# lks1248/SPH-EXA

Measured on AMD Instinct MI355X. Metric: particle-updates/sec (whole node), Sedov -n 400, 1/2/4/8 MI355X + HBM roofline %, higher is better.
Workload: dtype f32 hydro / f64 coordinates (sph::SphTypes)

## Files before the change

### sph-exa_amd/csrc/sx_sim.hpp

```cpp
#pragma once

#include <hip/hip_runtime.h>

#include <cmath>
#include <initializer_list>
#include <string>
#include <utility>
#include <vector>

#include "../../include/sphexa_hip.h"
#include "sx_comm.hpp"
#include "sx_hydro.hpp"
#include "sx_map.hpp"
#include "sx_profile.hpp"
#include "sx_fof.hpp"
#include "sx_twopoint.hpp"
#include "sx_spectrum.hpp"
#include "sx_step_timer.hpp"
#include "sx_tree.hpp"

namespace sx::turb
{
struct SimTurb;
}

namespace sx::sim
{

struct Scalars
{
    double   minDt, minDt_m1, ttot, minDtCourant, minDtRho;
    double   dtCand;
    float    courant;
    unsigned maxDivvU;
    double   egrav;
    unsigned long long maxAccSqBits;
    unsigned gravErr;
};

inline Scalars freshScalars(double minDt = 1e-6, double minDt_m1 = 1e-6)
{
    return Scalars{.minDt = minDt, .minDt_m1 = minDt_m1, .ttot = 0.0, .minDtCourant = INFINITY, .minDtRho = INFINITY,
                   .dtCand = 0.0, .courant = 1e10f, .maxDivvU = 0u, .egrav = 0.0, .maxAccSqBits = 0ull, .gravErr = 0u};
}

struct Fields
{
    double *  x, *y, *z, *temp;
    float *   h, *m, *vx, *vy, *vz, *xm1, *ym1, *zm1, *dum1, *alpha;
    uint64_t* id;
    uint8_t*  rung;
};

struct BdtState
{
    sx_timestep ts{}, prev{};
    bool        started{false};
    double      minDt{0}, minDt_m1{0}, ttot{0};
    float       searchExt{1.f};
    double      margin{1.05};
    double      egrav{0};
    uint64_t    haloShort{0};
    uint64_t    hierarchies{0}, warnedAt{~0ull};
    uint32_t*   groupBuf{nullptr};
    sx_groups   groups{}, tsGroups{}, active{}, rungs[SX_MAX_RUNGS]{};
    float*      groupDt{nullptr};
    uint32_t*   groupIdx{nullptr};
    uint32_t *  tsStart[2]{}, *tsEnd[2]{};
    uint8_t*    activeMask{nullptr};
    uint32_t*   maskRange{nullptr};
    uint64_t    substeps{0};
};

struct SkinState
{
    float    factor{0.05f};
    float    cur{0.05f};
    float    built{0.05f};
    int      maxReuse{24};
    float    staleLimit{0.125f};
    bool     valid{false};
    bool     forceBuild{false};
    int      sinceBuild{0};
    uint32_t ngmaxS{0};
    int      backoff{0}, backoffLen{4};
    int      cleanSinceBuild{0};
    uint64_t plainSteps{0};
    uint64_t builds{0}, reuseSteps{0}, staleClusters{0}, exactClusters{0};
    uint64_t resyncs{0};
    uint32_t lastStale{0}, lastExact{0};
    uint64_t stepClusters{0}, stepS13{0};
    bool      xmFused{false};
    uint32_t* exactList{nullptr};
    bool      listsKept{false};
    const void *keptNloc{nullptr}, *keptUni{nullptr}, *keptMask{nullptr}, *keptSame{nullptr}, *keptFrz{nullptr},
        *keptNlocB{nullptr};
    uint64_t  keptClusters{0}, frozenClusters{0};
    uint64_t  earlyExact{0};
    sx::ListsB lb{};
};


struct SkinBuffers
{
    float *   dx{nullptr}, *dy{nullptr}, *dz{nullptr};
    uint32_t* cells{nullptr};
    float *   rel{nullptr}, *hb{nullptr}, *acc{nullptr};
    uint32_t *sloc{nullptr}, *scnt{nullptr}, *ucountS{nullptr}, *l1{nullptr}, *l2{nullptr}, *l3{nullptr};
    uint8_t*  dec{nullptr};
    uint32_t* host{nullptr};
    uint8_t * streak{nullptr}, *same{nullptr};
    uint32_t* hitmask{nullptr};
    float2*   frz{nullptr};
    uint32_t *nlocB{nullptr}, *ucountB{nullptr}, *hitmaskB{nullptr};
    double *drift{nullptr}, *relg{nullptr}, *x0{nullptr}, *y0{nullptr}, *z0{nullptr};
    float* h0{nullptr};
};

struct ReqBox;

struct DomBuffers
{
    uint32_t* bins{nullptr};
    uint64_t *split{nullptr}, *seg{nullptr}, *cnth{nullptr};
    uint32_t *agree{nullptr}, *agreeh{nullptr};
    unsigned *hflag{nullptr}, *hflagh{nullptr};
    uint32_t* errh{nullptr};
    ReqBox*   mybox{nullptr};
};

struct GravBuffers
{
    unsigned long long* inter{nullptr};
    int32_t*            farL2N{nullptr};
    uint32_t*           farLay{nullptr};
};

}

struct sx_sim
{
    using Scalars = sx::sim::Scalars;
    using Fields  = sx::sim::Fields;

    sx_ctx*        ctx;
    sx::NsPolicy   nsPolicy;
    sx::Transport* comm{nullptr};
    sx_comm*       commHandle{nullptr};
    sx_params      p;
    sx_box         box;
    sx::DevBox     dbox;
    uint32_t       bucket;
    size_t         cap{0}, n{0}, first{0}, last{0};
    sx::Arena      mem;
    sx::Arena      work;
    sx::DevTree    tree;
    sx::DevTree    localTree;
    sx::Arena      farMem;
    sx::Arena      gravWork;
    sx::DevTree    farTree;
    sx::DevTree    nearTree;

    double *  x, *y, *z, *temp;
    float *   h, *m, *vx, *vy, *vz, *xm1, *ym1, *zm1, *dum1, *alpha;
    uint64_t* id;
    uint8_t*  rung{nullptr};
    uint64_t* keys;
    uint32_t *order, *nc;
    float *   xm, *kx, *gradh, *prho, *c, *divv, *curlv, *c11, *c12, *c13, *c22, *c23, *c33, *ax, *ay, *az;
    double*   du;
    float*    dV[6]{};
    float *   rho{nullptr}, *pres{nullptr};
    sx::RecX* rx;
    sx::RecV* rv;
    sx::RecT* rt;
    sx::RecS* rs;
    sx::RecC* rc;
    sx::NbLists nb;
    uint32_t* stats;
    uint32_t* statsHost;
    int       sortBits{30};
    bool      gravCount = false;
    uint32_t  gravCheckTargets{0};
    bool      gravCheckValid{false};
    double    gravCheck[6]{};
    bool      keysFresh = false;
    uint64_t  sortStats[4]{0, 0, 0, 0};
    Scalars*  sc;
    Scalars*  scHost;

    struct Spare
    {
        void** field;
        void*  alt;
        int    elemBytes;
    };
// ... 71 lines not shown
```

### sph-exa_amd/csrc/sx_sim_skin.cpp

```cpp
#include "sx_sim_internal.hpp"

using namespace sx;
using namespace sx::sim;

namespace
{

__global__ void coverListKernel(const uint32_t* list, uint32_t maxList, uint32_t first, uint32_t last, const double* x,
                                const double* y, const double* z, const float* r, float scale, const ReqBox* boxes,
                                DevBox box, double qmargin, const double* drift, const double* x0, const double* y0,
                                const double* z0, const double* relg, unsigned* flag)
{
    const uint32_t k = blockIdx.x;
    if (k >= min(list[0], maxList)) return;
    const uint32_t i = first + list[1 + k] * kCluster + threadIdx.x;
    if (i >= last) return;
    const ReqBox& b  = boxes[(i - first) / kChunk];
    const double  R  = 2.0 * (double)r[i] * (double)scale * (1.0 + 1e-6) + qmargin;
    const double  Ra = R + drift[0], Rr = R + relg[i];
    const bool    outNow = fabs(foldPbc(x[i] - b.c[0], box, 0)) + Ra > b.s[0] ||
                        fabs(foldPbc(y[i] - b.c[1], box, 1)) + Ra > b.s[1] ||
                        fabs(foldPbc(z[i] - b.c[2], box, 2)) + Ra > b.s[2];
    const bool    outBuild = fabs(foldPbc(x0[i] - b.c[0], box, 0)) + Rr > b.s[0] ||
                          fabs(foldPbc(y0[i] - b.c[1], box, 1)) + Rr > b.s[1] ||
// ... 58 lines not shown
void skinTooThin(SkinState& K)
{
    K.forceBuild = true;
    if (K.cur < kMaxSkin) K.cur = std::min(2.0f * K.cur, kMaxSkin);
    else
    {
        K.backoff    = K.backoffLen;
        K.backoffLen = std::min(2 * K.backoffLen, 32);
    }
}

SkinGrid skinGrid(const DevBox& b)
{
    SkinGrid g{};
    g.n = kSkinGridN;
    for (int d = 0; d < 3; ++d)
    {
        g.lo[d]  = b.lim[2 * d];
        g.inv[d] = (double)kSkinGridN / b.l[d];
        g.pbc[d] = b.pbc[d];
    }
    return g;
}

uint32_t skinCapacity(uint32_t ngmax, float factor)
{
    const double f = std::pow(1.0 + factor, 3.0) * 1.15;
    const uint32_t c = (uint32_t)std::ceil(ngmax * f);
    return std::min<uint32_t>(256u, (c + 1u) & ~1u);
}

static bool skinReserveDisp(sx_sim* s)
{
    auto& B = s->skinBuf;
    B.dx    = s->mem.get<float>("skin.dx", s->cap);
    B.dy    = s->mem.get<float>("skin.dy", s->cap);
    B.dz    = s->mem.get<float>("skin.dz", s->cap);
    B.cells = s->mem.get<uint32_t>("skin.cells", kGridWords * (size_t)kSkinGridN * kSkinGridN * kSkinGridN);
    return B.dx && B.dy && B.dz && B.cells;
}

static bool skinReserveDrift(sx_sim* s)
{
    auto& B = s->skinBuf;
    B.drift = s->mem.get<double>("skin.drift", 8);
    B.relg  = s->mem.get<double>("skin.relg", s->cap);
    B.x0    = s->mem.get<double>("skin.x0", s->cap);
    B.y0    = s->mem.get<double>("skin.y0", s->cap);
    B.z0    = s->mem.get<double>("skin.z0", s->cap);
    return B.drift && B.relg && B.x0 && B.y0 && B.z0;
}

bool skinParticleBuffers(sx_sim* s, PosArgs& q, hipStream_t st)
{
    const size_t nc = (size_t)kSkinGridN * kSkinGridN * kSkinGridN;
    const bool   ok = skinReserveDisp(s);
    const auto&  B  = s->skinBuf;
    q.dispX = B.dx, q.dispY = B.dy, q.dispZ = B.dz, q.cells = B.cells;
    q.grid  = skinGrid(s->dbox);
    if (!ok) return false;
    return hipMemsetAsync(q.cells, 0xff, 3 * nc * sizeof(uint32_t), st) == hipSuccess &&
           hipMemsetAsync(q.cells + 3 * nc, 0, 3 * nc * sizeof(uint32_t), st) == hipSuccess;
}

static bool skinReserveSearch(sx_sim* s, const NsArgs& na, uint32_t ncl, bool twoSets)
{
    auto&      B    = s->skinBuf;
    auto&      M    = s->mem;
    const bool disp = skinReserveDisp(s);
    B.rel     = M.get<float>("skin.rel", s->cap);
    B.sloc    = M.get<uint32_t>("skin.sloc", na.numGroups * (size_t)nlocWords(s->skin.ngmaxS) * kWave);
    B.scnt    = M.get<uint32_t>("skin.scnt", s->cap);
    B.hb      = M.get<float>("skin.hb", s->cap);
    B.acc     = M.get<float>("skin.acc", ncl);
    B.ucountS = M.get<uint32_t>("skin.ucount", ncl);
    B.l1      = M.get<uint32_t>("skin.l1", ncl + 1);
    B.l2      = M.get<uint32_t>("skin.l2", ncl + 1);
    B.l3      = M.get<uint32_t>("skin.l3", ncl + 1);
    B.dec     = M.get<uint8_t>("skin.dec", ncl);
    B.host    = M.pinned<uint32_t>("skin.host", 4);
    B.streak  = M.get<uint8_t>("skin.streak", ncl);
    B.hitmask = M.get<uint32_t>("skin.hitmask", na.numGroups * (size_t)kSkinMaskWords * kWave);
    B.same    = M.get<uint8_t>("skin.same", ncl);
    B.frz     = M.get<float2>("skin.frz", ncl);
    B.nlocB    = twoSets ? M.get<uint32_t>("skin.nlocB", na.numGroups * (size_t)nlocWords(na.ngmax) * kWave) : nullptr;
    B.ucountB  = twoSets ? M.get<uint32_t>("skin.ucountB", ncl) : nullptr;
    B.hitmaskB = twoSets ? M.get<uint32_t>("skin.hitmaskB", na.numGroups * (size_t)kSkinMaskWords * kWave) : nullptr;
    return disp && B.rel && B.sloc && B.scnt && B.hb && B.acc && B.ucountS && B.l1 && B.l2 && B.l3 && B.dec && B.host &&
           B.streak && B.hitmask && B.same && B.frz && (!twoSets || (B.nlocB && B.ucountB && B.hitmaskB));
}

int skinSearch(sx_sim* s, const NsArgs& na, bool reuse, hipStream_t st, float* xmOut, RecT* rtXm, SkinCounts& out)
{
    auto&          K   = s->skin;
    const uint32_t ncl = (na.numGroups + kClusterWaves - 1) / kClusterWaves;
    out                = SkinCounts{};
    out.clusters       = ncl;
    if (!reuse) K.built = K.cur;
    if (!ncl) return SX_OK;
    if (!reuse) K.ngmaxS = skinCapacity(s->p.ngmax, K.built);
    const bool twoSets = na.ucap / 4 >= (uint32_t)kSkinCap && !getenv("SX_SKIN_ONESET");
    if (!skinReserveSearch(s, na, ncl, twoSets)) return SX_ERR_NOMEM;
    const SkinBuffers& B = s->skinBuf;
    uint32_t *const l1 = B.l1, *const l2 = B.l2, *const l3 = B.l3, *const hl = B.host;
    uint32_t* const hmask = B.hitmask, *const nlocB = B.nlocB;
    uint8_t* const  same  = B.same;
    float2* const   frz   = B.frz;

    const SkinGrid g = skinGrid(s->dbox);
    SkinArgs fa{};
    fa.first = na.first, fa.last = na.last, fa.numGroups = na.numGroups, fa.ngmax = na.ngmax, fa.ng0 = na.ng0;
    fa.ngmaxS = K.ngmaxS, fa.iterateH = na.iterateH, fa.skin1 = 1.0f + K.built;
    fa.x = na.x, fa.y = na.y, fa.z = na.z, fa.h = na.h, fa.m = na.m, fa.nc = na.nc, fa.rxOut = na.rxOut;
    const uint32_t uoff = na.ucap / 2;
    fa.nloc = na.nloc, fa.uni = na.uni, fa.ucount = na.ucount, fa.ucap = na.ucap, fa.uoff = uoff, fa.ucountS = B.ucountS;
    fa.packMax = na.packMax;
    fa.sloc = B.sloc, fa.scnt = B.scnt, fa.hb = B.hb, fa.rel = B.rel, fa.acc = B.acc, fa.cells = B.cells, fa.grid = g;
    fa.dispX = B.dx, fa.dispY = B.dy, fa.dispZ = B.dz;
    fa.xmOut = xmOut, fa.rtXm = rtXm, fa.K = s->p.K;
    K.xmFused   = xmOut != nullptr;
    K.exactList = l2;
    fa.box = na.box, fa.powTab = na.powTab, fa.stats = na.stats, fa.clStats = na.clStats;
    fa.hitMask   = hmask;
    fa.same      = same;
    fa.nlocB = nlocB, fa.ucountB = B.ucountB, fa.hitMaskB = B.hitmaskB, fa.uoffB = na.ucap / 4;
    fa.frz       = getenv("SX_SKIN_NOFREEZE") ? nullptr : frz;
    fa.keepLists = reuse && K.listsKept && K.keptNloc == na.nloc && K.keptUni == na.uni && K.keptMask == hmask &&
                   K.keptSame == same && K.keptFrz == frz && K.keptNlocB == nlocB;
    K.listsKept  = false;

    NsArgs b   = na;
    b.skin1    = 1.0f + K.built;
    b.iterateH = 0;
    b.nloc     = B.sloc;
    b.packMax  = 0;
    b.ngmax    = K.ngmaxS;
    b.nc       = B.scnt;
    b.rxOut    = nullptr;
    b.uoff     = uoff;
    b.ucount   = B.ucountS;

    SIM_HIP(hipMemsetAsync(l1, 0, 4, st));
    SIM_HIP(hipMemsetAsync(l2, 0, 4, st));
    if (!reuse)
    {
        SIM_HIP(hipMemsetAsync(B.streak, 0, ncl, st));
        SIM_HIP(findNeighbors(b, st));
        fa.fresh = 1;
    }
    else fa.fresh = 0;
    fa.list  = nullptr;
    fa.stale = l1;
    fa.streak = reuse ? B.streak : nullptr;
    fa.direct = reuse ? l2 : nullptr;
    if (reuse)
    {
        fa.dec = B.dec;
        const char* fs = getenv("SX_SKIN_FROZEN_STAGE");
        fa.frozenStage = fs ? (uint32_t)std::max(0, atoi(fs)) : (uint32_t)kSkinFrozenCap;
        SIM_HIP(skinDecide(fa, ncl, st));
        SIM_HIP(skinFrozen(fa, ncl, st));
    }
    SIM_HIP(skinFilter(fa, ncl, st));
    SIM_HIP(hipMemcpyAsync(hl, l1, 4, hipMemcpyDeviceToHost, st));
    SIM_HIP(hipMemcpyAsync(hl + 1, l2, 4, hipMemcpyDeviceToHost, st));
    SIM_HIP(hipStreamSynchronize(st));
    const uint32_t n1 = hl[0], nd = hl[1];
    uint32_t       n2 = nd;
    out.rebuilt = n1, out.stale = n1 + nd, out.exact = nd;
    NsArgs         x  = na;
    NsPolicy large;
    large.mode = 1;
    if (reuse) b.policy = x.policy = &large;
    if ((n1 || nd) && reuse)
    {
        double* c3 = s->mem.get<double>("skin.centers", 3 * (size_t)s->tree.numNodes);
        double* s3 = s->mem.get<double>("skin.sizes", 3 * (size_t)s->tree.numNodes);
        if (!c3 || !s3) return SX_ERR_NOMEM;
        SIM_HIP(skinRefreshBoxes(s->tree, na.x, na.y, na.z, na.box, c3, s3, st));
        b.centers = x.centers = c3;
        b.sizes = x.sizes = s3;
    }
    const bool early = n1 && nd && reuse && s->auxStream && s->evAuxIn && s->evAuxOut && !getenv("SX_SKIN_SERIAL_EXACT");
    if (early)
    {
        NsArgs xd   = x;
        xd.subset   = l2;
        xd.work     = s->mem.get<uint32_t>("skin.aux.work", 16);
        xd.hSave    = s->mem.get<float>("skin.aux.over", ncl + 1);
        xd.hitMasks = s->mem.get<uint64_t>("skin.aux.masks", searchScratchBytes() / sizeof(uint64_t));
        const char* sh = getenv("SX_SKIN_AUX_SHARE");
        if (!sh || atoi(sh) != 0)
        {
            const unsigned G = searchGrid();
            xd.maxGrid       = std::min(nd, G / 2);
            b.maxGrid        = G - xd.maxGrid;
        }
        if (!xd.work || !xd.hSave || !xd.hitMasks) return SX_ERR_NOMEM;
        SIM_HIP(hipEventRecord(s->evAuxIn, st));
        SIM_HIP(hipStreamWaitEvent(s->auxStream, s->evAuxIn, 0));
        SIM_HIP(findNeighbors(xd, s->auxStream));
        SIM_HIP(hipEventRecord(s->evAuxOut, s->auxStream));
    }
    uint32_t* lx = l2;
    if (n1)
    {
        b.subset  = l1;
        SIM_HIP(findNeighbors(b, st));
        fa.fresh  = 1;
        fa.list   = l1;
        if (early) SIM_HIP(hipMemsetAsync(l3, 0, 4, st));
        fa.stale  = early ? l3 : l2;
        fa.streak = nullptr;
        fa.direct = nullptr;
        fa.dec    = nullptr;
        SIM_HIP(skinFilter(fa, ncl, st));
        SIM_HIP(hipMemcpyAsync(hl + 2, fa.stale, 4, hipMemcpyDeviceToHost, st));
        SIM_HIP(hipStreamSynchronize(st));
        n2 = hl[2];
    }
    uint32_t n3 = 0;
    if (early)
    {
        n3 = n2, n2 = nd + n3, lx = l3;
        K.earlyExact += nd;
        SIM_HIP(hipStreamWaitEvent(st, s->evAuxOut, 0));
    }
    out.exact = n2;
    {
        if (early ? n3 : n2)
        {
            x.subset = lx;
            SIM_HIP(findNeighbors(x, st));
        }
        if (early)
        {
            if (n3) SIM_HIP(hipMemcpyAsync(l2 + 1 + nd, l3 + 1, 4 * (size_t)n3, hipMemcpyDeviceToDevice, st));
            hl[3] = n2;
            SIM_HIP(hipMemcpyAsync(l2, hl + 3, 4, hipMemcpyHostToDevice, st));
        }
        if (n2)
        {
            if (reuse)
            {
                SIM_HIP(hipMemcpyAsync(hl, na.stats, 4, hipMemcpyDeviceToHost, st));
                SIM_HIP(hipStreamSynchronize(st));
                if (hl[0] & 1u)
                {
                    SIM_HIP(hipMemsetAsync(na.stats, 0, 4, st));
                    return kSkinResync;
                }
            }
            SIM_HIP(skinMarkStale(l2, ncl, B.acc, st));
        }
    }
    SIM_HIP(reduceClusterStats(na.clStats, ncl, na.stats, st));
    K.listsKept = true, K.keptNloc = na.nloc, K.keptUni = na.uni, K.keptMask = hmask, K.keptSame = same, K.keptFrz = frz;
    K.keptNlocB = nlocB;
    K.lb = twoSets ? ListsB{same, nlocB, B.ucountB, na.ucap / 4} : ListsB{};
    if (getenv("SX_SKIN_DEBUG"))
    {
        uint32_t f = 0;
        SIM_HIP(hipMemcpyAsync(&f, na.stats, 4, hipMemcpyDeviceToHost, st));
        SIM_HIP(hipStreamSynchronize(st));
        fprintf(stderr, "skin: reuse %d s %.3f clusters %u stale %u exact %u (direct %u) flags 0x%x mode %d\n",
                (int)reuse, K.built, ncl, n1 + nd, n2, nd, f, s->nsPolicy.mode);
    }
    return SX_OK;
}

void skinDecide(SkinState& K, bool reuse, const SkinCounts& c, uint64_t staleAll, uint64_t clustersAll)
{
    K.lastStale = c.stale, K.lastExact = c.exact;
    K.staleClusters += c.stale, K.exactClusters += c.exact;
    if (reuse)
    {
        K.reuseSteps++;
        K.sinceBuild++;
    }
    else
    {
        K.builds++;
        K.valid      = true;
        K.forceBuild = false;
        K.sinceBuild = 0;
    }
    const bool clean = (double)staleAll <= K.staleLimit * (double)clustersAll;
    if (!reuse) K.cleanSinceBuild = 0;
    else if (clean) K.cleanSinceBuild++;
    if (!clean)
    {
        K.forceBuild = true;
        if (!reuse || K.cleanSinceBuild < 2) skinTooThin(K);
        else if (K.sinceBuild < kShortSkin) K.cur = std::min(1.25f * K.cur, kMaxSkin);
    }
    if (clean && K.cleanSinceBuild >= 2) K.backoffLen = 4;
}

int skinHaloRefresh(sx_sim* s, hipStream_t st)
{
    if (int e = haloExchange(s, {{s->x, 8}, {s->y, 8}, {s->z, 8}, {s->h, 4}, {s->m, 4}}, st)) return e;
    const size_t nc = (size_t)kSkinGridN * kSkinGridN * kSkinGridN;
    const auto&  B  = s->skinBuf;
    if (!skinReserveDisp(s)) return SX_ERR_NOMEM;
    SIM_COMM(s->comm->allreduceMinU32(B.cells, 3 * nc, st));
    SIM_COMM(s->comm->allreduceMaxU32(B.cells + 3 * nc, 3 * nc, st));
    if (!skinReserveDrift(s)) return SX_ERR_NOMEM;
    uint32_t* red = reinterpret_cast<uint32_t*>(B.drift + 2);
    SIM_HIP(hipMemsetAsync(red, 0, 7 * 4, st));
    SIM_HIP(hipMemsetAsync(red + 1, 0xff, 3 * 4, st));
    skinGridMaxKernel<<<grid(nc), 256, 0, st>>>(B.cells, (uint32_t)nc, red);
    const size_t nl = s->last - s->first;
    skinDriftKernel<<<std::max(1u, grid(nl)), 256, 0, st>>>(red, (uint32_t)s->first, (uint32_t)s->last, B.dx, B.dy, B.dz,
                                                           B.drift, B.relg);
    SIM_HIP(hipGetLastError());
    return SX_OK;
}

int skinBuildSnapshot(sx_sim* s, hipStream_t st)
{
    if (!skinReserveDrift(s)) return SX_ERR_NOMEM;
    const auto&  B  = s->skinBuf;
    const size_t f0 = s->first, nl0 = s->last - s->first;
    SIM_HIP(hipMemsetAsync(B.drift, 0, 8 * sizeof(double), st));
    SIM_HIP(hipMemsetAsync(B.relg + f0, 0, nl0 * sizeof(double), st));
    double*       p0[3] = {B.x0, B.y0, B.z0};
    const double* pc[3] = {s->x, s->y, s->z};
    for (int d = 0; d < 3; ++d)
        SIM_HIP(hipMemcpyAsync(p0[d] + f0, pc[d] + f0, nl0 * sizeof(double), hipMemcpyDeviceToDevice, st));
    return SX_OK;
}

int skinCoverCheck(sx_sim* s, const SkinCounts& c, unsigned* flag, hipStream_t st)
{
    const auto& B = s->skinBuf;
    if (!B.drift || !B.relg || !B.x0 || !B.y0 || !B.z0) return SX_ERR_NOMEM;
    const double   qm    = quantMargin(s->dbox);
    const uint32_t first = (uint32_t)s->first, last = (uint32_t)s->last;
    if (c.rebuilt)
        coverListKernel<<<c.rebuilt, kCluster, 0, st>>>(B.l1, c.rebuilt, first, last, s->x, s->y, s->z, B.hb,
                                                        1.0f + s->skin.built, s->dom.mybox, s->dbox, qm, B.drift, B.x0,
// ... 18 lines not shown
```

### sph-exa_amd/csrc/sx_skin.hip

```cpp
#include "sx_kernel_poly.hpp"
#include "sx_skin.hpp"
#include "sx_traverse.hpp"

namespace sx
{

namespace
{

constexpr int kWalkPF  = 8;
constexpr int kWalkBlocks = (nlocWords(256) + kWalkPF - 1) / kWalkPF;
constexpr int kB       = kCluster;

__device__ __forceinline__ int cellIndex(double v, const SkinGrid& g, int d) { return gridCell(v, g, d); }

__device__ __forceinline__ float keepOrZero(float v, bool k)
{
    return __builtin_bit_cast(float, __builtin_bit_cast(uint32_t, v) & (0u - (uint32_t)k));
}

__device__ __forceinline__ float norm3up(float x, float y, float z)
{
    return sqrtf(fmaf(x, x, fmaf(y, y, z * z))) * (1.0f + 0x1p-18f) + 1e-30f;
}
// ... 65 lines not shown
    {
        centers[3 * node + d] = gc[3 * node + d] + 0.5 * (lo[d] + hi[d]);
        sizes[3 * node + d]   = 0.5 * (hi[d] - lo[d]);
    }
}

__global__ void markStaleKernel(const uint32_t* list, uint32_t numClusters, float* acc)
{
    const uint32_t k = blockIdx.x * blockDim.x + threadIdx.x;
    if (k < list[0] && k < numClusters) acc[list[1 + k]] = INFINITY;
}

__global__ __launch_bounds__(1024) void reduceClusterStatsKernel(const uint4* cl, uint32_t n, uint32_t* stats)
{
    __shared__ uint32_t           s_max[4][16];
    __shared__ unsigned long long s_sum[3][16];
    uint32_t                      mx = 0, mu = 0, kp = 0, fz = 0;
    unsigned long long            st = 0, te = 0, un = 0;
    for (uint32_t i = threadIdx.x; i < n; i += blockDim.x)
    {
        const uint4 v = cl[i];
        mx = max(mx, v.x), st += v.y & 0x3fffffffu, te += v.z, un += v.w, mu = max(mu, v.w), kp += v.y >> 31,
        fz += (v.y >> 30) & 1u;
    }
    mx = waveMax(mx), mu = waveMax(mu), st = waveSum(st), te = waveSum(te), un = waveSum(un), kp = waveSum(kp), fz = waveSum(fz);
    const int w = threadIdx.x >> 6;
    if ((threadIdx.x & 63) == 0)
        s_max[0][w] = mx, s_max[1][w] = mu, s_max[2][w] = kp, s_max[3][w] = fz, s_sum[0][w] = st, s_sum[1][w] = te, s_sum[2][w] = un;
    __syncthreads();
    if (threadIdx.x == 0)
    {
        for (int k = 1; k < (int)(blockDim.x >> 6); ++k)
            mx = max(mx, s_max[0][k]), mu = max(mu, s_max[1][k]), kp += s_max[2][k], fz += s_max[3][k], st += s_sum[0][k],
            te += s_sum[1][k], un += s_sum[2][k];
        stats[2]                                          = mx;
        stats[18]                                         = kp;
        stats[19]                                         = fz;
        stats[12]                                         = mu;
        *reinterpret_cast<unsigned long long*>(stats + 4) = st;
        *reinterpret_cast<unsigned long long*>(stats + 6) = te;
        *reinterpret_cast<unsigned long long*>(stats + 8) = un;
    }
}

__device__ __forceinline__ void pushStale(const SkinArgs& a, uint32_t c)
{
    uint32_t* L = (a.direct && a.streak && a.streak[c]) ? a.direct : a.stale;
    L[1 + atomicAdd(&L[0], 1u)] = c;
    if (a.streak) a.streak[c] = 1;
    if (a.same) a.same[c] = 0;
}
static_assert((kWalkBlocks + 1) / 2 <= (int)kSkinMaskWords, "hit-mask words per target");

__device__ __forceinline__ uint32_t listState(const SkinArgs& a, uint32_t c)
{
    return (a.same && a.keepLists && !a.fresh) ? (uint32_t)a.same[c] : 0u;
}

__global__ __launch_bounds__(kB) void skinDecideKernel(SkinArgs a)
{
    __shared__ float s_red[kClusterWaves];
    __shared__ int   s_vote[kClusterWaves];

    const uint32_t c    = blockIdx.x;
    const int      wave = __builtin_amdgcn_readfirstlane(threadIdx.x >> 6), lane = threadIdx.x & 63;
    const uint32_t gw   = c * kClusterWaves + wave;
    const uint32_t c0   = a.first + c * kCluster;
    const uint32_t i    = c0 + threadIdx.x;
    const bool     valid = gw < a.numGroups && i < a.last;
    const uint32_t iS    = valid ? i : c0;
    const double   xi = a.x[iS], yi = a.y[iS], zi = a.z[iS];
    const double   ox = a.x[c0], oy = a.y[c0], oz = a.z[c0];
    const float    hi  = a.h[iS];
    const float    hbi = a.hb[iS];
    const float    ux = a.dispX[c0], uy = a.dispY[c0], uz = a.dispZ[c0];
    const float    di = a.rel[iS] + norm3up(a.dispX[iS] - ux, a.dispY[iS] - uy, a.dispZ[iS] - uz);
    const float    Ri = 2.0f * (hbi * a.skin1);
    const uint32_t scount = valid ? a.scnt[i] - 1u : 0u;
    const uint32_t U      = __builtin_amdgcn_readfirstlane(a.ucountS[c]);
    const float    kEps   = 0x1p-16f;
    const uint32_t lstate    = listState(a, c);
    const uint32_t lcur      = (a.nlocB && (lstate & kListsBSel)) ? 1u : 0u;
    const bool     mayFreeze = a.frz && ((lstate >> lcur) & 1u) != 0;
    const float2   fref      = mayFreeze ? a.frz[c] : make_float2(-INFINITY, -INFINITY);

    const double rx = foldPbc(xi - ox, a.box, 0), ry = foldPbc(yi - oy, a.box, 1), rz = foldPbc(zi - oz, a.box, 2);
    double       lo[3]  = {valid ? rx : INFINITY, valid ? ry : INFINITY, valid ? rz : INFINITY};
    double       hb3[3] = {valid ? rx : -INFINITY, valid ? ry : -INFINITY, valid ? rz : -INFINITY};
    float        rmax   = valid ? Ri : 0.0f;
    for (int d = 0; d < 3; ++d)
    {
        lo[d]  = -waveMax(-lo[d]);
        hb3[d] = waveMax(hb3[d]);
    }
    rmax      = waveMax(rmax);
    float gmx = 0.0f;
    if (rmax > 0.0f)
    {
        const double o[3] = {ox, oy, oz};
        int          k0[3], nk[3];
        uint32_t     total = 1;
        for (int d = 0; d < 3; ++d)
        {
            k0[d]  = cellIndex(o[d] + lo[d] - (double)rmax, a.grid, d);
            int k1 = cellIndex(o[d] + hb3[d] + (double)rmax, a.grid, d);
            nk[d]  = k1 - k0[d] + 1;
            if (a.grid.pbc[d] && nk[d] >= a.grid.n) k0[d] = 0, nk[d] = a.grid.n;
            total *= nk[d];
        }
        for (uint32_t q = lane; q < total; q += kWave)
        {
            int      k[3];
            uint32_t r = q;
            for (int d = 0; d < 3; ++d)
            {
                const uint32_t rq = r / (uint32_t)nk[d];
                k[d]              = k0[d] + (int)(r - rq * (uint32_t)nk[d]);
                r                 = rq;
                if (a.grid.pbc[d]) k[d] = wrapCell(k[d], a.grid.n);
            }
            const size_t nc   = (size_t)a.grid.n * a.grid.n * a.grid.n;
            const size_t cell = ((size_t)k[2] * a.grid.n + k[1]) * a.grid.n + k[0];
            const uint32_t lx = a.cells[cell], ly = a.cells[nc + cell], lz = a.cells[2 * nc + cell];
            if (lx != 0xffffffffu)
            {
                const float ex = fmaxf(fabsf(orderedFloat(lx) - ux), fabsf(orderedFloat(a.cells[3 * nc + cell]) - ux));
                const float ey = fmaxf(fabsf(orderedFloat(ly) - uy), fabsf(orderedFloat(a.cells[4 * nc + cell]) - uy));
                const float ez = fmaxf(fabsf(orderedFloat(lz) - uz), fabsf(orderedFloat(a.cells[5 * nc + cell]) - uz));
                gmx = fmaxf(gmx, norm3up(ex, ey, ez));
            }
        }
    }
    gmx = waveMax(gmx);
    if (lane == 0) s_red[wave] = gmx;
    __syncthreads();
    float g = s_red[0];
    for (int w = 1; w < kClusterWaves; ++w)
        g = fmaxf(g, s_red[w]);
    const float A = a.acc[c] + g;

    const bool bad = valid && (scount > a.ngmaxS || !(2.0f * hi + di + A <= Ri * (1.0f - kEps)));
    const bool thin = valid && 2.0f * hi + 2.0f * (di + A) > Ri * (1.0f - kEps);
    const float e    = di + A + kEps * Ri;
    const bool  melt = valid && !(e + 2.0f * hi < fref.x && e - 2.0f * hi < fref.y);
    uint32_t w = 0;
    w |= __ballot(bad) != 0 ? 1u : 0u;
    w |= __ballot(thin) != 0 ? 2u : 0u;
    w |= __ballot(melt) != 0 ? 4u : 0u;
    if (lane == 0) s_vote[wave] = (int)w;
    __syncthreads();
    uint32_t v = 0;
    for (int k = 0; k < kClusterWaves; ++k)
        v |= (uint32_t)s_vote[k];
    if ((v & 1u) || U > (uint32_t)kSkinCap || U > a.ucap - a.uoff)
    {
        if (threadIdx.x == 0)
        {
            pushStale(a, c);
            a.dec[c] = kSkinStale;
        }
        return;
    }
    if (valid) a.rel[i] = di;
    if (threadIdx.x == 0)
    {
        if (v & 2u) atomicAdd(&a.stats[13], 1u);
        a.acc[c] = A;
        a.dec[c] = (mayFreeze && !(v & 4u)) ? kSkinFrozen : kSkinWalk;
    }
}

__global__ __launch_bounds__(kB) __attribute__((amdgpu_waves_per_eu(6))) void skinFrozenKernel(SkinArgs a)
{
    __shared__ float4 s_rec[kSkinFrozenCap];
    __shared__ uint4  s_cst[kClusterWaves];

    const uint32_t c = xcdBlock(blockIdx.x, gridDim.x);
    if (a.dec[c] != kSkinFrozen) return;
    const int      wave = __builtin_amdgcn_readfirstlane(threadIdx.x >> 6), lane = threadIdx.x & 63;
    const uint32_t gw   = c * kClusterWaves + wave;
    const uint32_t c0   = a.first + c * kCluster;
    const uint32_t i    = c0 + threadIdx.x;
    const bool     valid = gw < a.numGroups && i < a.last;
    const uint32_t iS    = valid ? i : c0;
    const double   xi = a.x[iS], yi = a.y[iS], zi = a.z[iS];
    const double   ox = a.x[c0], oy = a.y[c0], oz = a.z[c0];
    const float    hi = a.h[iS], mi = a.m[iS];
    const uint32_t count  = valid ? a.nc[i] - 1u : 0u;
    const uint32_t stored = min(count, a.ngmax);
    const uint32_t scount = valid ? a.scnt[i] - 1u : 0u;
    const bool      setB = a.nlocB && (a.same[c] & kListsBSel);
    const uint32_t* ll   = (setB ? a.nlocB : a.nloc) + (size_t)gw * nlocWords(a.ngmax) * kWave + lane;
    const uint32_t* un   = a.uni + (size_t)c * a.ucap + (setB ? a.uoffB : 0u);
    const uint32_t  ue   = __builtin_amdgcn_readfirstlane(setB ? a.ucountB[c] : a.ucount[c]);
    float           rho0 = mi;
    const uint32_t  cap  = min(a.frozenStage, (uint32_t)kSkinFrozenCap);
    if (a.xmOut)
    {
        const float xr = (float)foldPbc(xi - ox, a.box, 0), yr = (float)foldPbc(yi - oy, a.box, 1),
                    zr = (float)foldPbc(zi - oz, a.box, 2);
        auto record = [&](uint32_t j) {
            return make_float4((float)foldPbc(a.x[j] - ox, a.box, 0), (float)foldPbc(a.y[j] - oy, a.box, 1),
                               (float)foldPbc(a.z[j] - oz, a.box, 2), a.m[j]);
        };
        {
            constexpr int  S = 4;
            const uint32_t ns = min(ue, cap);
#pragma unroll 1
            for (uint32_t u0 = threadIdx.x; u0 < ns; u0 += S * kB)
            {
                uint32_t js[S];
#pragma unroll
                for (int q = 0; q < S; ++q)
                    js[q] = un[min(u0 + q * kB, ns - 1u)];
                double px[S], py[S], pz[S];
                float  mq[S];
#pragma unroll
                for (int q = 0; q < S; ++q)
                    px[q] = a.x[js[q]], py[q] = a.y[js[q]], pz[q] = a.z[js[q]], mq[q] = a.m[js[q]];
#pragma unroll
                for (int q = 0; q < S; ++q)
                    if (u0 + q * kB < ns)
                        s_rec[u0 + q * kB] = make_float4((float)foldPbc(px[q] - ox, a.box, 0), (float)foldPbc(py[q] - oy, a.box, 1),
                                                         (float)foldPbc(pz[q] - oz, a.box, 2), mq[q]);
            }
            __syncthreads();
        }
        const float hInv = 1.0f / hi, hInv2 = hInv * hInv;
        auto term = [&](uint32_t p, bool k) {
            const float4 q  = s_rec[min(p, (uint32_t)kSkinFrozenCap - 1u)];
            const float  dx = q.x - xr, dy = q.y - yr, dz = q.z - zr;
            const float  r2 = fmaf(dx, dx, fmaf(dy, dy, dz * dz));
            rho0 += keepOrZero(kernelWt(r2 * hInv2) * q.w, k);
        };
        const bool staged = ue <= cap;
        if (valid && staged && ue <= a.packMax)
        {
            const uint32_t  ngr = p12::groups(stored), lastG = ngr ? ngr - 1 : 0u;
            const uint32_t* lp  = ll + (p12::kWords - 1) * lane;
            constexpr int   PW  = 2 * p12::kWords;
            auto            lw  = [&](uint32_t g0, int u) {
                return lp[(size_t)min(g0 + u / p12::kWords, lastG) * (p12::kWords * kWave) + u % p12::kWords];
            };
            uint32_t nx[PW];
#pragma unroll
            for (int u = 0; u < PW; ++u)
                nx[u] = lw(0, u);
            for (uint32_t g0 = 0; g0 < ngr; g0 += 2)
            {
                uint32_t cw[PW];
#pragma unroll
                for (int u = 0; u < PW; ++u)
                {
                    cw[u] = nx[u];
                    nx[u] = lw(g0 + 2, u);
                }
#pragma unroll
                for (int h2 = 0; h2 < 2; ++h2)
                {
                    const uint32_t w0 = cw[3 * h2], w1 = cw[3 * h2 + 1], w2 = cw[3 * h2 + 2];
                    const uint32_t pos[8] = {p12::get<0>(w0, w1, w2), p12::get<1>(w0, w1, w2), p12::get<2>(w0, w1, w2),
                                             p12::get<3>(w0, w1, w2), p12::get<4>(w0, w1, w2), p12::get<5>(w0, w1, w2),
                                             p12::get<6>(w0, w1, w2), p12::get<7>(w0, w1, w2)};
#pragma unroll
                    for (uint32_t e = 0; e < 8; ++e)
                        term(pos[e], 8 * (g0 + h2) + e < stored);
                }
            }
        }
        else if (valid && staged)
        {
            const uint32_t nw = (stored + 1) >> 1, last = nw ? nw - 1 : 0u;
            constexpr int  PF = kWalkPF;
            uint32_t       nx[PF];
#pragma unroll
            for (int u = 0; u < PF; ++u)
                nx[u] = ll[(size_t)min((uint32_t)u, last) * kWave];
            for (uint32_t w0 = 0; w0 < nw; w0 += PF)
            {
                uint32_t cw[PF];
#pragma unroll
                for (int u = 0; u < PF; ++u)
                {
                    cw[u] = nx[u];
                    nx[u] = ll[(size_t)min(w0 + PF + u, last) * kWave];
                }
#pragma unroll
                for (int u = 0; u < PF; ++u)
                {
                    term(cw[u] & 0xffffu, 2 * (w0 + u) < stored);
                    term(cw[u] >> 16, 2 * (w0 + u) + 1 < stored);
                }
            }
        }
        else if (valid)
        {
#pragma unroll 1
            for (uint32_t e = 0; e < stored; ++e)
            {
                uint32_t p;
                if (ue <= a.packMax)
                {
                    const uint32_t* g = ll + (p12::kWords - 1) * lane + (size_t)(e / p12::kGroup) * (p12::kWords * kWave);
                    const uint32_t  w[p12::kWords] = {g[0], g[1], g[2]};
                    p                              = p12::get(w, e % p12::kGroup);
                }
                else
                {
                    const uint32_t w = ll[(size_t)(e >> 1) * kWave];
                    p                = (e & 1u) ? w >> 16 : w & 0xffffu;
                }
                const float4 q  = p < cap ? s_rec[p] : record(un[min(p, ue - 1u)]);
                const float  dx = q.x - xr, dy = q.y - yr, dz = q.z - zr;
                const float  r2 = fmaf(dx, dx, fmaf(dy, dy, dz * dz));
                rho0 += kernelWt(r2 * hInv2) * q.w;
            }
        }
    }

    if (valid)
    {
        if (a.rxOut) a.rxOut[i] = RecX{xi, yi, zi, hi, mi};
        if (a.xmOut)
        {
            const float hInv  = 1.0f / hi;
            const float h3Inv = hInv * hInv * hInv;
            const float xm    = (float)((double)mi / ((double)rho0 * a.K * (double)h3Inv));
            a.xmOut[i]        = xm;
            if (a.rtXm) a.rtXm[i] = RecT{xm, 0.0f, 0.0f, 0.0f};
        }
    }
    const uint32_t maxCnt = waveMax(count), nst = waveSum(stored), walked = waveSum(scount);
    if (lane == 0) s_cst[wave] = make_uint4(maxCnt, nst, walked, 0u);
    __syncthreads();
    if (threadIdx.x == 0)
    {
        uint4 t = s_cst[0];
        for (int w = 1; w < kClusterWaves; ++w)
            t.x = max(t.x, s_cst[w].x), t.y += s_cst[w].y, t.z += s_cst[w].z;
        t.y |= 0xc0000000u;
        t.w          = ue;
        a.clStats[c] = t;
        if (a.streak) a.streak[c] = 0;
    }
}

__global__ __launch_bounds__(kB) __attribute__((amdgpu_waves_per_eu(4))) void skinFilterKernel(SkinArgs a,
                                                                                              uint32_t numClusters)
{
    __shared__ float4   s_rec[kSkinCap];
    __shared__ uint8_t  s_hit[kSkinCap + 4];
    __shared__ uint16_t s_bm[kWalkBlocks][kB];
    uint16_t* const     s_rank = reinterpret_cast<uint16_t*>(s_rec);
    __shared__ float    s_red[kClusterWaves];
    __shared__ int      s_vote[kClusterWaves];
    __shared__ uint32_t s_wsum[kClusterWaves];
    __shared__ uint4    s_cst[kClusterWaves];

    const uint32_t nWork = a.list ? __builtin_amdgcn_readfirstlane(a.list[0]) : numClusters;
    if (blockIdx.x >= nWork) return;
    const uint32_t blk  = a.list ? blockIdx.x : xcdBlock(blockIdx.x, gridDim.x);
    const uint32_t c    = __builtin_amdgcn_readfirstlane(a.list ? a.list[1 + blk] : blk);
    if (a.dec && a.dec[c] != kSkinWalk) return;
    const int      wave = __builtin_amdgcn_readfirstlane(threadIdx.x >> 6), lane = threadIdx.x & 63;
    const uint32_t gw   = c * kClusterWaves + wave;
    const uint32_t c0   = a.first + c * kCluster;
    const uint32_t i    = c0 + threadIdx.x;
    const bool     valid = gw < a.numGroups && i < a.last;
    const uint32_t iS    = valid ? i : c0;
    const double   xi = a.x[iS], yi = a.y[iS], zi = a.z[iS];
    const double   ox = a.x[c0], oy = a.y[c0], oz = a.z[c0];
    float          hi   = a.h[iS];
    const float    h0   = hi;
    const float    hbi  = a.fresh ? hi : a.hb[iS];
    const float    di = a.fresh ? 0.0f : a.rel[iS];
    const float    A  = a.fresh ? 0.0f : a.acc[c];
    const float    Ri = 2.0f * (hbi * a.skin1);
    const uint32_t scount = valid ? a.scnt[i] - 1u : 0u;
    const uint32_t U      = __builtin_amdgcn_readfirstlane(a.ucountS[c]);
    const float    kEps   = 0x1p-16f;
    const uint32_t lstate   = listState(a, c);
    const uint32_t lcur     = (a.nlocB && (lstate & kListsBSel)) ? 1u : 0u;
    const bool     curValid = ((lstate >> lcur) & 1u) != 0;
    auto blockAny = [&](bool v) -> bool {
        const int w = __ballot(v) != 0;
        if (lane == 0) s_vote[wave] = w;
        __syncthreads();
        int any = 0;
        for (int k = 0; k < kClusterWaves; ++k)
            any |= s_vote[k];
        __syncthreads();
        return any != 0;
    };

    auto withinSkin = [&](float h) { return 2.0f * h + di + A <= Ri * (1.0f - kEps); };
    if (a.fresh && (blockAny(valid && (scount > a.ngmaxS || !withinSkin(hi))) || U > (uint32_t)kSkinCap ||
                    U > a.ucap - a.uoff))
    {
        if (threadIdx.x == 0) pushStale(a, c);
        return;
    }
    int      iteration = 0;
    unsigned count = 0, stored = 0;
    const float mi   = a.m[iS];
// ... 227 lines not shown
            const uint32_t t = __shfl_up(incl, o, kWave);
            if (lane >= o) incl += t;
        }
        if (lane == kWave - 1) s_wsum[wave] = incl;
        __syncthreads();
        uint32_t run = incl - sum;
        for (int w = 0; w < wave; ++w)
            run += s_wsum[w];
        for (int w = 0; w < kClusterWaves; ++w)
            ue += s_wsum[w];
        uint32_t* ux = setUnion(ltgt);
        for (uint32_t u0 = b0; u0 < b1; u0 += 8)
        {
            uint32_t jj[8];
#pragma unroll
            for (int q = 0; q < 8; ++q)
                jj[q] = un[min(u0 + q, U - 1u)];
#pragma unroll
            for (int q = 0; q < 8; ++q)
                if (u0 + q < b1)
                {
                    s_rank[u0 + q] = (uint16_t)run;
                    if (s_hit[u0 + q]) ux[run++] = jj[q];
                }
        }
        __syncthreads();
    }
    if (!kept && ue <= a.packMax)
    {
        uint32_t* lw = setLists(ltgt) + (p12::kWords - 1) * lane;
        uint32_t  acc = 0, nb = 0, t = 0, n = 0, lastR = 0, bits = 0;
        auto      push = [&](uint32_t r, bool keep) {
            acc |= keep ? r << nb : 0u;
            nb += keep ? p12::kBits : 0u;
            n += keep ? 1u : 0u;
            if (nb >= 32u)
            {
                lw[t] = acc;
                nb -= 32u;
                acc = r >> (p12::kBits - nb);
                if (++t == p12::kWords) t = 0, lw += p12::kWords * kWave;
            }
        };
        walk([&](uint32_t b) { bits = s_bm[b][threadIdx.x]; },
             [&](uint32_t p, int e, bool) {
                 const bool keep = ((bits >> e) & 1u) != 0;
                 lastR           = keep ? s_rank[p] : lastR;
                 push(lastR, keep);
             },
             [](uint32_t) {});
        while (n & (p12::kGroup - 1u))
            push(lastR, true);
        if (uint32_t* const hm = setMask(ltgt))
            for (uint32_t k = 0; 2 * k < nbl; ++k)
                hm[(size_t)k * kWave] = maskWord(k);
        if (threadIdx.x == 0) *setCount(ltgt) = ue;
    }
    else if (!kept)
    {
        uint32_t* const lw = setLists(ltgt);
        unsigned st = 0;
        uint32_t pend = 0, bits = 0;
        walk([&](uint32_t b) { bits = s_bm[b][threadIdx.x]; },
             [&](uint32_t p, int e, bool) {
                 const bool     keep = ((bits >> e) & 1u) != 0;
                 const uint32_t r    = s_rank[p];
                 const bool     odd  = (st & 1u) != 0;
                 if (keep && odd) lw[(size_t)(st >> 1) * kWave] = pend | (r << 16);
                 pend = (keep && !odd) ? r : pend;
                 st += keep ? 1u : 0u;
             },
             [](uint32_t) {});
        if (st & 1u) lw[(size_t)(st >> 1) * kWave] = pend;
        if (uint32_t* const hm = setMask(ltgt))
            for (uint32_t k = 0; 2 * k < nbl; ++k)
                hm[(size_t)k * kWave] = maskWord(k);
        if (threadIdx.x == 0) *setCount(ltgt) = ue;
    }
    if (threadIdx.x == 0 && a.same && lnew != lstate) a.same[c] = (uint8_t)lnew;

    if (valid)
    {
        a.nc[i] = count + 1;
        if (a.iterateH && iteration > 0) a.h[i] = hi;
        if (a.rxOut) a.rxOut[i] = RecX{xi, yi, zi, hi, a.m[i]};
        if (a.fresh) a.hb[i] = h0, a.rel[i] = 0.0f;
        if (a.xmOut)
        {
            const float hInv  = 1.0f / hi;
            const float h3Inv = hInv * hInv * hInv;
            const float xm    = (float)((double)mi / ((double)rho0 * a.K * (double)h3Inv));
            a.xmOut[i]        = xm;
            if (a.rtXm) a.rtXm[i] = RecT{xm, 0.0f, 0.0f, 0.0f};
        }
    }
    if (threadIdx.x == 0)
    {
        if (a.fresh) a.acc[c] = 0.0f;
        if (a.streak && !a.fresh) a.streak[c] = 0;
    }
    const unsigned           failed = (valid && a.iterateH && iteration >= 10) ? 1u : 0u;
    const unsigned           nfail  = waveSum(failed);
    const unsigned           maxCnt = waveMax(valid ? count : 0u);
    const unsigned long long nst    = waveSum((unsigned long long)(valid ? stored : 0u));
    const unsigned long long walked = waveSum((unsigned long long)scount);
    const float kp = waveMin(valid ? frzK + 2.0f * hi : INFINITY), km = waveMin(valid ? frzK - 2.0f * hi : INFINITY);
    if (lane == 0)
    {
        if (nfail) atomicAdd(&a.stats[1], nfail);
        s_cst[wave]  = make_uint4(maxCnt, (uint32_t)nst, (uint32_t)walked, __float_as_uint(kp));
        s_wsum[wave] = __float_as_uint(km);
    }
    __syncthreads();
    if (threadIdx.x == 0)
    {
        if (a.frz)
        {
            float2 f = make_float2(__uint_as_float(s_cst[0].w), __uint_as_float(s_wsum[0]));
            for (int w = 1; w < kClusterWaves; ++w)
                f.x = fminf(f.x, __uint_as_float(s_cst[w].w)), f.y = fminf(f.y, __uint_as_float(s_wsum[w]));
            a.frz[c] = f;
        }
        uint4 t = s_cst[0];
        for (int w = 1; w < kClusterWaves; ++w)
            t.x = max(t.x, s_cst[w].x), t.y += s_cst[w].y, t.z += s_cst[w].z;
        t.y |= kept ? 0x80000000u : 0u;
        t.w          = ue;
        a.clStats[c] = t;
    }
}

inline unsigned grid1(size_t n, int b = 256) { return (unsigned)((n + b - 1) / b); }

}

hipError_t skinDecide(const SkinArgs& a, uint32_t numClusters, hipStream_t s)
{
    if (numClusters) skinDecideKernel<<<numClusters, kB, 0, s>>>(a);
    return hipGetLastError();
}

hipError_t skinFrozen(const SkinArgs& a, uint32_t numClusters, hipStream_t s)
{
    if (numClusters) skinFrozenKernel<<<numClusters, kB, 0, s>>>(a);
    return hipGetLastError();
}

hipError_t skinFilter(const SkinArgs& a, uint32_t numClusters, hipStream_t s)
{
    if (numClusters) skinFilterKernel<<<numClusters, kB, 0, s>>>(a, numClusters);
    return hipGetLastError();
}

hipError_t skinRefreshBoxes(const DevTree& t, const double* x, const double* y, const double* z, const DevBox& box,
                            double* centers, double* sizes, hipStream_t s, bool withCells)
{
    if (t.numNodes <= 0) return hipSuccess;
    leafBoxKernel<<<grid1(t.numNodes, 16), 256, 0, s>>>(t.childOffsets, t.internalToLeaf, t.layout, t.numNodes,
                                                          t.centers, t.sizes, x, y, z, box, centers, sizes,
                                                          withCells ? 1 : 0);
    for (int level = kMaxLevel; level >= 0; --level)
    {
        const int b = t.levelRangeHost[level], e = t.levelRangeHost[level + 1];
        if (e > b) innerBoxKernel<<<grid1(e - b), 256, 0, s>>>(t.childOffsets, b, e, t.centers, box, centers, sizes);
    }
    return hipGetLastError();
}

hipError_t skinMarkStale(const uint32_t* list, uint32_t numClusters, float* acc, hipStream_t s)
{
    if (numClusters) markStaleKernel<<<grid1(numClusters), 256, 0, s>>>(list, numClusters, acc);
    return hipGetLastError();
}

hipError_t reduceClusterStats(const uint4* clStats, uint32_t numClusters, uint32_t* stats, hipStream_t s)
{
    reduceClusterStatsKernel<<<1, 1024, 0, s>>>(clStats, numClusters, stats);
    return hipGetLastError();
}

}
```

### sph-exa_amd/csrc/sx_skin.hpp

```cpp
#pragma once

#include "sx_tree.hpp"

namespace sx
{

using SkinGrid = DispGrid;

constexpr int kSkinGridN = 64;
constexpr int kSkinCap   = 1920;
constexpr uint32_t kSkinMaskWords = 8;

struct SkinArgs
{
    uint32_t first, last, numGroups, ngmax, ng0;
    uint32_t ngmaxS;
    int      iterateH;
    int      fresh;
    float    skin1;
    const double *x, *y, *z;
    float*       h;
    const float* m;
    uint32_t*    nc;
    RecX*        rxOut;
    uint32_t*       nloc;
    uint32_t        packMax;
    uint32_t*       uni;
    uint32_t*       ucount;
    uint32_t        ucap;
    uint32_t        uoff;
    const uint32_t* ucountS;
    const uint32_t* sloc;
    const uint32_t* scnt;
    float*          hb;
    float*          rel;
    const float *   dispX, *dispY, *dispZ;
    float*          acc;
    const uint32_t* cells;
    SkinGrid        grid;
    const uint32_t* list;
    uint32_t*       stale;
    uint8_t*        dec;
    uint32_t        frozenStage;
    uint8_t*        streak;
    uint32_t*       direct;
    uint32_t*       hitMask;
    uint8_t*        same;
    int             keepLists;
    uint32_t*       nlocB;
    uint32_t*       ucountB;
    uint32_t*       hitMaskB;
    uint32_t        uoffB;
    float2*         frz;
    DevBox          box;
    const float*    powTab;
    float*          xmOut;
    RecT*           rtXm;
    double          K;
    uint32_t*       stats;
    uint4*          clStats;
};

constexpr int kSkinFrozenCap = 1664;

constexpr uint8_t kSkinStale = 0, kSkinFrozen = 1, kSkinWalk = 2;

hipError_t skinDecide(const SkinArgs& a, uint32_t numClusters, hipStream_t s);
hipError_t skinFrozen(const SkinArgs& a, uint32_t numClusters, hipStream_t s);
hipError_t skinFilter(const SkinArgs& a, uint32_t numClusters, hipStream_t s);
hipError_t skinRefreshBoxes(const DevTree& t, const double* x, const double* y, const double* z, const DevBox& box,
                            double* centers, double* sizes, hipStream_t s, bool withCells = false);
hipError_t skinMarkStale(const uint32_t* list, uint32_t numClusters, float* acc, hipStream_t s);
hipError_t reduceClusterStats(const uint4* clStats, uint32_t numClusters, uint32_t* stats, hipStream_t s);

}
```

Measured before the change: 1.155 billion.

## Let skin clusters freeze onto the alternate kept neighbor list set

Stores a freeze reference and per-particle neighbor counts for both kept list sets (A and B). When the current set fails its freeze test, the decide kernel checks the other set and, if it still covers the cluster, switches the cluster's list selector and routes it to the frozen path instead of a full walk. The frozen kernel then restores nc from the saved per-set count. This aims to cut neighbor-walk work in exchange for extra memory (a uint16 count array, a doubled frz buffer) and more complex list-state bookkeeping.

```diff
diff --git a/sph-exa_amd/csrc/sx_sim.hpp b/sph-exa_amd/csrc/sx_sim.hpp
--- a/sph-exa_amd/csrc/sx_sim.hpp
+++ b/sph-exa_amd/csrc/sx_sim.hpp
@@ -94,7 +94,7 @@
     uint32_t* exactList{nullptr};
     bool      listsKept{false};
     const void *keptNloc{nullptr}, *keptUni{nullptr}, *keptMask{nullptr}, *keptSame{nullptr}, *keptFrz{nullptr},
-        *keptNlocB{nullptr};
+        *keptNlocB{nullptr}, *keptCnt{nullptr};
     uint64_t  keptClusters{0}, frozenClusters{0};
     uint64_t  earlyExact{0};
     sx::ListsB lb{};
@@ -112,6 +112,7 @@
     uint8_t * streak{nullptr}, *same{nullptr};
     uint32_t* hitmask{nullptr};
     float2*   frz{nullptr};
+    uint16_t* cnt{nullptr};
     uint32_t *nlocB{nullptr}, *ucountB{nullptr}, *hitmaskB{nullptr};
     double *drift{nullptr}, *relg{nullptr}, *x0{nullptr}, *y0{nullptr}, *z0{nullptr};
     float* h0{nullptr};
diff --git a/sph-exa_amd/csrc/sx_sim_skin.cpp b/sph-exa_amd/csrc/sx_sim_skin.cpp
--- a/sph-exa_amd/csrc/sx_sim_skin.cpp
+++ b/sph-exa_amd/csrc/sx_sim_skin.cpp
@@ -164,12 +164,13 @@
     B.streak  = M.get<uint8_t>("skin.streak", ncl);
     B.hitmask = M.get<uint32_t>("skin.hitmask", na.numGroups * (size_t)kSkinMaskWords * kWave);
     B.same    = M.get<uint8_t>("skin.same", ncl);
-    B.frz     = M.get<float2>("skin.frz", ncl);
+    B.frz     = M.get<float2>("skin.frz", 2 * (size_t)ncl);
+    B.cnt     = M.get<uint16_t>("skin.cnt", 2 * (size_t)s->cap);
     B.nlocB    = twoSets ? M.get<uint32_t>("skin.nlocB", na.numGroups * (size_t)nlocWords(na.ngmax) * kWave) : nullptr;
     B.ucountB  = twoSets ? M.get<uint32_t>("skin.ucountB", ncl) : nullptr;
     B.hitmaskB = twoSets ? M.get<uint32_t>("skin.hitmaskB", na.numGroups * (size_t)kSkinMaskWords * kWave) : nullptr;
     return disp && B.rel && B.sloc && B.scnt && B.hb && B.acc && B.ucountS && B.l1 && B.l2 && B.l3 && B.dec && B.host &&
-           B.streak && B.hitmask && B.same && B.frz && (!twoSets || (B.nlocB && B.ucountB && B.hitmaskB));
+           B.streak && B.hitmask && B.same && B.frz && B.cnt && (!twoSets || (B.nlocB && B.ucountB && B.hitmaskB));
 }
 
 int skinSearch(sx_sim* s, const NsArgs& na, bool reuse, hipStream_t st, float* xmOut, RecT* rtXm, SkinCounts& out)
@@ -207,8 +208,10 @@
     fa.same      = same;
     fa.nlocB = nlocB, fa.ucountB = B.ucountB, fa.hitMaskB = B.hitmaskB, fa.uoffB = na.ucap / 4;
     fa.frz       = getenv("SX_SKIN_NOFREEZE") ? nullptr : frz;
+    fa.cnt       = B.cnt;
+    fa.freezeOther = getenv("SX_SKIN_FREEZE_CURRENT") ? 0 : 1;
     fa.keepLists = reuse && K.listsKept && K.keptNloc == na.nloc && K.keptUni == na.uni && K.keptMask == hmask &&
-                   K.keptSame == same && K.keptFrz == frz && K.keptNlocB == nlocB;
+                   K.keptSame == same && K.keptFrz == frz && K.keptNlocB == nlocB && K.keptCnt == B.cnt;
     K.listsKept  = false;
 
     NsArgs b   = na;
@@ -338,7 +341,7 @@
     }
     SIM_HIP(reduceClusterStats(na.clStats, ncl, na.stats, st));
     K.listsKept = true, K.keptNloc = na.nloc, K.keptUni = na.uni, K.keptMask = hmask, K.keptSame = same, K.keptFrz = frz;
-    K.keptNlocB = nlocB;
+    K.keptNlocB = nlocB, K.keptCnt = B.cnt;
     K.lb = twoSets ? ListsB{same, nlocB, B.ucountB, na.ucap / 4} : ListsB{};
     if (getenv("SX_SKIN_DEBUG"))
     {
diff --git a/sph-exa_amd/csrc/sx_skin.hip b/sph-exa_amd/csrc/sx_skin.hip
--- a/sph-exa_amd/csrc/sx_skin.hip
+++ b/sph-exa_amd/csrc/sx_skin.hip
@@ -171,7 +171,12 @@
     const uint32_t lstate    = listState(a, c);
     const uint32_t lcur      = (a.nlocB && (lstate & kListsBSel)) ? 1u : 0u;
     const bool     mayFreeze = a.frz && ((lstate >> lcur) & 1u) != 0;
-    const float2   fref      = mayFreeze ? a.frz[c] : make_float2(-INFINITY, -INFINITY);
+    const bool     maySwitch = a.frz && a.nlocB && a.freezeOther && ((lstate >> (1u - lcur)) & 1u) != 0;
+    const float4   fboth     = a.frz ? reinterpret_cast<const float4*>(a.frz)[c] : make_float4(0.0f, 0.0f, 0.0f, 0.0f);
+    const float2   fref      = mayFreeze ? (lcur ? make_float2(fboth.z, fboth.w) : make_float2(fboth.x, fboth.y))
+                                         : make_float2(-INFINITY, -INFINITY);
+    const float2   foth      = maySwitch ? (lcur ? make_float2(fboth.x, fboth.y) : make_float2(fboth.z, fboth.w))
+                                         : make_float2(-INFINITY, -INFINITY);
 
     const double rx = foldPbc(xi - ox, a.box, 0), ry = foldPbc(yi - oy, a.box, 1), rz = foldPbc(zi - oz, a.box, 2);
     double       lo[3]  = {valid ? rx : INFINITY, valid ? ry : INFINITY, valid ? rz : INFINITY};
@@ -232,10 +237,12 @@
     const bool thin = valid && 2.0f * hi + 2.0f * (di + A) > Ri * (1.0f - kEps);
     const float e    = di + A + kEps * Ri;
     const bool  melt = valid && !(e + 2.0f * hi < fref.x && e - 2.0f * hi < fref.y);
+    const bool  meltO = valid && !(e + 2.0f * hi < foth.x && e - 2.0f * hi < foth.y);
     uint32_t w = 0;
     w |= __ballot(bad) != 0 ? 1u : 0u;
     w |= __ballot(thin) != 0 ? 2u : 0u;
     w |= __ballot(melt) != 0 ? 4u : 0u;
+    w |= __ballot(meltO) != 0 ? 8u : 0u;
     if (lane == 0) s_vote[wave] = (int)w;
     __syncthreads();
     uint32_t v = 0;
@@ -255,7 +262,9 @@
     {
         if (v & 2u) atomicAdd(&a.stats[13], 1u);
         a.acc[c] = A;
-        a.dec[c] = (mayFreeze && !(v & 4u)) ? kSkinFrozen : kSkinWalk;
+        const bool frozen = mayFreeze && !(v & 4u), switched = !frozen && maySwitch && !(v & 8u);
+        if (switched) a.same[c] = (uint8_t)(lstate ^ kListsBSel);
+        a.dec[c] = frozen ? kSkinFrozen : (switched ? kSkinFrozenSwitch : kSkinWalk);
     }
 }
 
@@ -265,7 +274,9 @@
     __shared__ uint4  s_cst[kClusterWaves];
 
     const uint32_t c = xcdBlock(blockIdx.x, gridDim.x);
-    if (a.dec[c] != kSkinFrozen) return;
+    const uint32_t dec = a.dec[c];
+    if (dec != kSkinFrozen && dec != kSkinFrozenSwitch) return;
+    const bool     sw   = dec == kSkinFrozenSwitch;
     const int      wave = __builtin_amdgcn_readfirstlane(threadIdx.x >> 6), lane = threadIdx.x & 63;
     const uint32_t gw   = c * kClusterWaves + wave;
     const uint32_t c0   = a.first + c * kCluster;
@@ -275,10 +286,10 @@
     const double   xi = a.x[iS], yi = a.y[iS], zi = a.z[iS];
     const double   ox = a.x[c0], oy = a.y[c0], oz = a.z[c0];
     const float    hi = a.h[iS], mi = a.m[iS];
-    const uint32_t count  = valid ? a.nc[i] - 1u : 0u;
+    const bool      setB = a.nlocB && (a.same[c] & kListsBSel);
+    const uint32_t count  = valid ? (sw ? (uint32_t)a.cnt[2 * (size_t)i + (setB ? 1u : 0u)] : a.nc[i]) - 1u : 0u;
     const uint32_t stored = min(count, a.ngmax);
     const uint32_t scount = valid ? a.scnt[i] - 1u : 0u;
-    const bool      setB = a.nlocB && (a.same[c] & kListsBSel);
     const uint32_t* ll   = (setB ? a.nlocB : a.nloc) + (size_t)gw * nlocWords(a.ngmax) * kWave + lane;
     const uint32_t* un   = a.uni + (size_t)c * a.ucap + (setB ? a.uoffB : 0u);
     const uint32_t  ue   = __builtin_amdgcn_readfirstlane(setB ? a.ucountB[c] : a.ucount[c]);
@@ -409,6 +420,7 @@
 
     if (valid)
     {
+        if (sw) a.nc[i] = count + 1;
         if (a.rxOut) a.rxOut[i] = RecX{xi, yi, zi, hi, mi};
         if (a.xmOut)
         {
@@ -802,6 +814,7 @@
     if (valid)
     {
         a.nc[i] = count + 1;
+        if (a.cnt) a.cnt[2 * (size_t)i + ltgt] = (uint16_t)(count + 1);
         if (a.iterateH && iteration > 0) a.h[i] = hi;
         if (a.rxOut) a.rxOut[i] = RecX{xi, yi, zi, hi, a.m[i]};
         if (a.fresh) a.hb[i] = h0, a.rel[i] = 0.0f;
@@ -839,7 +852,7 @@
             float2 f = make_float2(__uint_as_float(s_cst[0].w), __uint_as_float(s_wsum[0]));
             for (int w = 1; w < kClusterWaves; ++w)
                 f.x = fminf(f.x, __uint_as_float(s_cst[w].w)), f.y = fminf(f.y, __uint_as_float(s_wsum[w]));
-            a.frz[c] = f;
+            a.frz[2 * (size_t)c + ltgt] = f;
         }
         uint4 t = s_cst[0];
         for (int w = 1; w < kClusterWaves; ++w)
diff --git a/sph-exa_amd/csrc/sx_skin.hpp b/sph-exa_amd/csrc/sx_skin.hpp
--- a/sph-exa_amd/csrc/sx_skin.hpp
+++ b/sph-exa_amd/csrc/sx_skin.hpp
@@ -52,6 +52,8 @@
     uint32_t*       hitMaskB;
     uint32_t        uoffB;
     float2*         frz;
+    int             freezeOther;
+    uint16_t*       cnt;
     DevBox          box;
     const float*    powTab;
     float*          xmOut;
@@ -63,7 +65,7 @@
 
 constexpr int kSkinFrozenCap = 1664;
 
-constexpr uint8_t kSkinStale = 0, kSkinFrozen = 1, kSkinWalk = 2;
+constexpr uint8_t kSkinStale = 0, kSkinFrozen = 1, kSkinWalk = 2, kSkinFrozenSwitch = 3;
 
 hipError_t skinDecide(const SkinArgs& a, uint32_t numClusters, hipStream_t s);
 hipError_t skinFrozen(const SkinArgs& a, uint32_t numClusters, hipStream_t s);
```

New measurement: 1.109 billion. -4.0%, worse.
